# Shizheng-Wen/GAOT-3D

Hardware: AMD Instinct MI355X
Metric: mesh-points/sec fwd+bwd, 500K-pt DrivAerNet++ sample (higher is better)
Workload: dtype bf16; 1 GPU; configs[1]: one 500000-point car-like surface sample, latent 64x64x32, knn k=8 encoder + flipped decoder, C=32 P=2 d=256 h=8 F=1024 L=10 rope, attention dropout 0.1 (training mode), MSE + AdamW step; CSR build and geoembed stats inside the step (a decoder list that is the encoder's with its rows swapped shares the encoder's two lists); points=500000, edges=4000000, edges_decoder=4000000, layers=10, precision=bf16, points_per_gpu=500000, point_order=random

## Files before the change

gaot_3d_amd/csrc/gno.hip:

```cpp
#include <type_traits>

#include "gno_common.h"

namespace {

using namespace gno;

template <int NH, int H>
struct FwdLds {
    static constexpr int KB = H / 32;
    static constexpr int w0 = 0;
    static constexpr int b0 = w0 + IN0P * H;
    static constexpr int wl = b0 + H;
    static constexpr int wL = wl + (NH - 1) * (H * H + H);
    static constexpr int bL = wL + H * 32;
    static constexpr int weights_end = bL + 32;
};

template <int NH, int H, int T, int MODE, class... Nl>
__global__ __launch_bounds__(256, 2) void k_gno_fwd(MlpPtrs mlp, const float* __restrict__ y_pos,
                                                    const float* __restrict__ x_pos, const float* __restrict__ f_y,
                                                    const int* __restrict__ src_s, const int* __restrict__ dst_s,
                                                    const int* __restrict__ rowptr, int64_t E, float* __restrict__ out,
                                                    float* __restrict__ part, Nl... nl_) {
// ... 131 lines not shown
                    acc = __builtin_amdgcn_mfma_f32_32x32x2f32(h[t][kb][r], b, acc, 0, 0, 0);
                }
#pragma unroll
            for (int r = 0; r < 16; ++r) {
                const int el = mfma32_row(r, hf);
                if constexpr (MODE == MODE_KERNELONLY) {
                    stage[(t * 32 + el) * C + l31] = acc[r];
                } else {
                    const int s = ids[(t * 2 + 0) * 32 + el];
                    const float fv = f_y[(int64_t)s * C + l31];
                    stage[(t * 32 + el) * C + l31] = acc[r] * fv;
                }
            }
        }
        wave_lds_fence();
        if (hf < T) {
            segment_walk<C>(stage + hf * 32 * C, C, ids + (hf * 2 + 1) * 32, l31, base + 32 * hf, rowptr, out, part,
                            true);
        }
        wave_lds_fence();
    }
}

__global__ void k_scale_by_inv_deg(const float* __restrict__ gout, const int* __restrict__ rowptr, int64_t Q,
                                   float* __restrict__ gs) {
    const int64_t i = (int64_t)blockIdx.x * blockDim.x + threadIdx.x;
    if (i >= Q * 8) return;
    const int64_t q = i >> 3;
    const int deg = rowptr[q + 1] - rowptr[q];
    const float inv = deg > 0 ? 1.0f / (float)deg : 0.f;
    float4 v = reinterpret_cast<const float4*>(gout)[i];
    reinterpret_cast<float4*>(gs)[i] = make_float4(v.x * inv, v.y * inv, v.z * inv, v.w * inv);
}

__global__ void k_transpose_w(const float* __restrict__ w, int out_dim, int in_dim, float* __restrict__ wt) {
    const int i = blockIdx.x * blockDim.x + threadIdx.x;
    if (i >= out_dim * in_dim) return;
    const int j = i / in_dim, k = i % in_dim;
    wt[k * out_dim + j] = w[i];
}

template <int NH, int H>
struct ParamLayout {
    static constexpr int C = 32;
    static constexpr int w_off(int l) { return l == 0 ? 0 : (H * IN0 + H) + (l - 1) * (H * H + H); }
    static constexpr int b_off(int l) { return w_off(l) + (l == 0 ? H * IN0 : (l == NH ? C * H : H * H)); }
    static constexpr int total = (H * IN0 + H) + (NH - 1) * (H * H + H) + (C * H + C);
};

template <int B, int E, class F>
__device__ __forceinline__ void static_for(F&& f) {
    if constexpr (B < E) {
        f(std::integral_constant<int, B>{});
        static_for<B + 1, E>(f);
    }
}

struct WRsrc {
    __amdgpu_buffer_rsrc_t w[GAOT_MAX_MLP_LAYERS];
    __amdgpu_buffer_rsrc_t wt[GAOT_MAX_MLP_LAYERS];
};
__device__ __forceinline__ float bload(__amdgpu_buffer_rsrc_t r, int voff, int soff) {
// ... 360 lines not shown
        for (int r = 0; r < 16; ++r) wp[PL::w_off(NH) + mfma32_row(r, hf) * H + 32 * wave + l31] = dWL[r];
#pragma unroll
        for (int r = 0; r < 16; ++r)
            if (l31 < IN0) wp[PL::w_off(0) + (32 * wave + mfma32_row(r, hf)) * IN0 + l31] = dW0[r];
        const float t0 = db0 + __shfl_xor(db0, 32, 64);
        if (hf == 0) wp[PL::b_off(0) + 32 * wave + l31] = t0;
        if (wave == 0) {
            const float tl = dbL + __shfl_xor(dbL, 32, 64);
            if (hf == 0) wp[PL::b_off(NH) + l31] = tl;
        }
    }
#pragma unroll
    for (int l = 1; l < NH; ++l) {
#pragma unroll
        for (int r = 0; r < 16; ++r)
            wp[PL::w_off(l) + (32 * wjb + mfma32_row(r, hf)) * H + 32 * wkb + l31] = dWh[l - 1][r];
        if (wkb == 0) {
            const float t = dbh[l - 1] + __shfl_xor(dbh[l - 1], 32, 64);
            if (hf == 0) wp[PL::b_off(l) + 32 * wjb + l31] = t;
        }
    }
}

__global__ __launch_bounds__(256) void k_reduce_params(const float* __restrict__ wpart, int n_waves, int total,
                                                       float* __restrict__ flat) {
    __shared__ float red[4][64];
    const int o = threadIdx.x & 63, sl = threadIdx.x >> 6;
    const int p = blockIdx.x * 64 + o;
    float s = 0.f;
    if (p < total)
        for (int w = sl; w < n_waves; w += 4) s += wpart[(int64_t)w * total + p];
    red[sl][o] = s;
    __syncthreads();
    if (sl == 0 && p < total) flat[p] = ((red[0][o] + red[1][o]) + red[2][o]) + red[3][o];
}

struct ScatterDesc {
    float* dst[2 * GAOT_MAX_MLP_LAYERS];
    int off[2 * GAOT_MAX_MLP_LAYERS + 1];
    int n;
};
__global__ void k_scatter_params(const float* __restrict__ flat, ScatterDesc d) {
    const int p = blockIdx.x * blockDim.x + threadIdx.x;
    if (p >= d.off[d.n]) return;
    int t = 0;
    while (p >= d.off[t + 1]) ++t;
    d.dst[t][p - d.off[t]] = flat[p];
}

int param_total(int nh, int h) { return (h * IN0 + h) + (nh - 1) * (h * h + h) + (32 * h + 32); }

size_t fwd_lds_bytes(int nh, int h, int t) {
    const int weights = IN0P * h + h + (nh - 1) * (h * h + h) + h * 32 + 32;
    return sizeof(float) * (size_t)(weights + 4 * t * 32 * 32) + sizeof(int) * (size_t)(4 * t * 2 * 32);
}
size_t bwd_lds_bytes(int nh, int h, bool coords = false) {
    const int per_wave = nh * 32 * (h + 1) + 32 * (h + 1) + 32 * IN0P + 64;
    return sizeof(float) * (size_t)(4 * per_wave + nh * h + 32 + (coords ? IN0 * h : 0));
}

template <int NH, int H, int MODE>
int launch_fwd(const MlpPtrs& p, const float* y_pos, const float* x_pos, const float* f_y, const float* ttab, const int* src_s,
               const int* dst_s, const int* rowptr, int64_t E, float* out, float* part, hipStream_t st) {
    constexpr int T = 2;
    const size_t lds = fwd_lds_bytes(NH, H, T);
    auto kern = [] {
        if constexpr (MODE == MODE_LINEAR) return k_gno_fwd<NH, H, T, MODE>;
        else return k_gno_fwd<NH, H, T, MODE, NlFwd>;
    }();
    hipError_t e = hipFuncSetAttribute((const void*)kern, hipFuncAttributeMaxDynamicSharedMemorySize, (int)lds);
// ... 45 lines not shown
                               rowptr_src, E, grad_f, part, wpart, nl);
    }
    return GAOT_OK;
}

int bwd_grid(int64_t E) {
    const int64_t n_tiles = ceil_div(E, 32);
    return (int)std::max<int64_t>(1, std::min<int64_t>(ceil_div(n_tiles, 4), 256));
}

bool mlp_supported(const gaot_mlp_t* m, bool backward, int precision = 0) {
    return m && m->channels == 32 && (m->hidden == 64) && m->n_hidden >= 1 &&
           m->n_hidden <= (backward ? (precision == 1 ? 4 : 3) : 4);
}

}

int gaot_gno_fwd_bf16_dispatch(int n_hidden, int mode, const float* const* w, const float* const* b, const float* y_pos,
                               const float* x_pos, const float* f_y, const float* ttab, const int32_t* src_sorted,
                               const int32_t* dst_sorted, const int32_t* rowptr_dst, int64_t num_edges, float* out, float* part,
                               hipStream_t st);

size_t gaot_gno_bwd_bf16_image_bytes(int n_hidden);
int gaot_gno_bwd_bf16_dispatch(int n_hidden, int mode, const float* const* w, const float* const* b, const float* w0t,
                               void* images, const float* y_pos, const float* x_pos, const float* f_y, const float* gs,
                               const int32_t* src_sorted, const int32_t* dst_sorted, const int32_t* rowptr_src,
                               int64_t num_edges, float* grad_f, float* part, float* wpart, float* gcoord, const float* ttab,
                               float* dt, float* part_dt, int grid, hipStream_t st);

extern "C" size_t gaot_gno_fwd_workspace_bytes(int64_t num_edges, int channels) {
    return sizeof(float) * (size_t)(ceil_div(num_edges, 32) * 2 * channels) + 64;
}

namespace {
#define GNO_CHECK(cond, msg)                              \
    do {                                                  \
        if (!(cond)) {                                    \
            gaot_set_error("%s: %s", fn, msg);            \
            return GAOT_ERR_ARG;                          \
        }                                                 \
    } while (0)
int gno_fwd_impl(const char* fn, const gaot_mlp_t* mlp, const float* y_pos, const float* x_pos, const float* f_y,
                 const float* ttab, int mode, const int32_t* src_sorted, const int32_t* dst_sorted, const int32_t* rowptr_dst,
                 int64_t num_edges, int64_t num_queries, float* out, int precision, void* workspace, size_t workspace_bytes,
                 gaot_stream_t stream) {
    GNO_CHECK(mlp, "null mlp");
    if (!mlp_supported(mlp, false)) {
        gaot_set_error("%s: unsupported MLP shape (n_hidden=%d hidden=%d channels=%d)", fn, mlp->n_hidden,
// ... 14 lines not shown
    float* part = (float*)workspace;
    int rc = GAOT_OK;
    if (num_edges > 0) {
        GNO_CHECK(y_pos && x_pos && (f_y || mode == MODE_KERNELONLY) && src_sorted && dst_sorted, "null pointer");
        GNO_CHECK(mode == MODE_LINEAR || ttab, "null t");
        GNO_CHECK(precision == 0 || precision == 1, "precision must be 0 (fp32) or 1 (bf16 matrix cores)");
        if (precision == 1) {
            rc = gaot_gno_fwd_bf16_dispatch(mlp->n_hidden, mode, p.w, p.b, y_pos, x_pos, f_y, ttab, src_sorted, dst_sorted,
                                            rowptr_dst, num_edges, out, part, st);
        } else {
#define GNO_FWD_CASE(NH_, MODE_)                                                                                          \
    case NH_ * 3 + MODE_:                                                                                                 \
        rc = launch_fwd<NH_, 64, MODE_>(p, y_pos, x_pos, f_y, ttab, src_sorted, dst_sorted, rowptr_dst, num_edges, out, part, st); \
        break;
#define GNO_FWD_CASES(NH_) GNO_FWD_CASE(NH_, MODE_LINEAR) GNO_FWD_CASE(NH_, MODE_NONLINEAR) GNO_FWD_CASE(NH_, MODE_KERNELONLY)
            switch (mlp->n_hidden * 3 + mode) {
                GNO_FWD_CASES(1) GNO_FWD_CASES(2) GNO_FWD_CASES(3) GNO_FWD_CASES(4)
            }
#undef GNO_FWD_CASES
#undef GNO_FWD_CASE
        }
        if (rc != GAOT_OK) return rc;
    }
    const int64_t n = num_queries * 8;
    GAOT_KLAUNCH((k_segment_fixup<32>), dim3(segment_fixup_grid(n)), dim3(256), 0, st, rowptr_dst,
                       num_queries, part, out, 1);
    GAOT_LAUNCH_CHECK();
    return GAOT_OK;
}
}

extern "C" int gaot_gno_fwd(const gaot_mlp_t* mlp, const float* y_pos, const float* x_pos, const float* f_y,
                            const int32_t* src_sorted, const int32_t* dst_sorted, const int32_t* rowptr_dst,
                            int64_t num_edges, int64_t num_queries, float* out, int precision, void* workspace,
                            size_t workspace_bytes, gaot_stream_t stream) {
    GAOT_ENTER();
    return gno_fwd_impl("gaot_gno_fwd", mlp, y_pos, x_pos, f_y, nullptr, MODE_LINEAR, src_sorted, dst_sorted, rowptr_dst,
                        num_edges, num_queries, out, precision, workspace, workspace_bytes, stream);
}

extern "C" int gaot_gno_fwd_nl(const gaot_mlp_t* mlp, int mode, const float* y_pos, const float* x_pos, const float* f_y,
                               const float* src_table, const int32_t* src_sorted, const int32_t* dst_sorted,
                               const int32_t* rowptr_dst, int64_t num_edges, int64_t num_queries, float* out, int precision,
                               void* workspace, size_t workspace_bytes, gaot_stream_t stream) {
    GAOT_ENTER();
    GAOT_CHECK_ARG(mode == MODE_NONLINEAR || mode == MODE_KERNELONLY, "mode must be 1 (nonlinear) or 2 (nonlinear_kernelonly)");
    return gno_fwd_impl("gaot_gno_fwd_nl", mlp, y_pos, x_pos, f_y, src_table, mode, src_sorted, dst_sorted, rowptr_dst,
                        num_edges, num_queries, out, precision, workspace, workspace_bytes, stream);
// ... 25 lines not shown
    GNO_CHECK(mlp && grads, "null mlp");
    if (!mlp_supported(mlp, true, precision)) {
        gaot_set_error("%s: unsupported MLP shape (n_hidden=%d hidden=%d channels=%d; four hidden layers in bf16 mode only)", fn,
                       mlp->n_hidden, mlp->hidden, mlp->channels);
        return GAOT_ERR_UNSUPPORTED;
    }
    GNO_CHECK(num_edges >= 0 && num_sources >= 0 && num_queries >= 0, "negative size");
    GNO_CHECK(precision != 1 || (num_sources <= (1 << 24) && num_queries <= (1 << 24)),
                   "bf16 GNO backward: more than 2^24 source or query rows (run the mesh point-sharded or in fp32 mode)");
    GNO_CHECK(precision != 1 || num_edges < ((int64_t)1 << 27),
                   "bf16 GNO backward: 2^27 or more edges in one launch (run the mesh point-sharded or in fp32 mode)");
    const bool nlm = mode != MODE_LINEAR;
    GNO_CHECK(workspace_bytes >= (nlm ? gaot_gno_bwd_nl_workspace_bytes(mlp, num_edges, num_queries)
                                      : gaot_gno_bwd_workspace_bytes(mlp, num_edges, num_queries)), "workspace too small");
    GNO_CHECK(rowptr_src && rowptr_dst, "null rowptr");
    GNO_CHECK(!nlm || num_sources == 0 || dt, "null grad_src_table");
    hipStream_t st = (hipStream_t)stream;
    const int nh = mlp->n_hidden, h = mlp->hidden;
    const int total = param_total(nh, h);
    const int grid = bwd_grid(num_edges);
    const int n_waves = grid;
    float* part = (float*)workspace;
    float* wt = part + ceil_div(num_edges, 16) * 2 * 32;
    float* flat = wt + total;
    float* wpart = flat + total;
    float* gs = wpart + (size_t)grid * total;
    void* images = (void*)(((uintptr_t)(gs + (size_t)num_queries * 32) + 255) & ~(uintptr_t)255);
    float* part_dt = (float*)(((uintptr_t)images + gaot_gno_bwd_bf16_image_bytes(nh) + 255) & ~(uintptr_t)255);
    GNO_CHECK(precision == 0 || precision == 1, "precision must be 0 (fp32) or 1 (bf16 matrix cores)");

    MlpPtrs p, pt;
    int off = 0;
    for (int l = 0; l <= nh; ++l) {
        p.w[l] = mlp->weight[l];
        p.b[l] = mlp->bias[l];
        GNO_CHECK(p.w[l] && p.b[l] && grads->weight[l] && grads->bias[l], "null MLP parameter / gradient");
        const int out_dim = (l == nh) ? 32 : h;
        const int in_dim = (l == 0) ? IN0 : h;
        pt.w[l] = wt + off;
        pt.b[l] = p.b[l];
        if (num_edges > 0)
            GAOT_KLAUNCH(k_transpose_w, dim3((unsigned)ceil_div(out_dim * in_dim, 256)), dim3(256), 0, st, p.w[l],
                               out_dim, in_dim, wt + off);
        off += out_dim * in_dim;
    }
    ScatterDesc sd;
    sd.n = 2 * (nh + 1);
    {
        int o = 0;
        for (int l = 0; l <= nh; ++l) {
            const int out_dim = (l == nh) ? 32 : h;
            const int in_dim = (l == 0) ? IN0 : h;
            sd.dst[2 * l] = grads->weight[l];
            sd.off[2 * l] = o;
            o += out_dim * in_dim;
            sd.dst[2 * l + 1] = grads->bias[l];
            sd.off[2 * l + 1] = o;
            o += out_dim;
        }
        sd.off[sd.n] = o;
    }
    const bool want_gf = mode != MODE_KERNELONLY;
    if (num_edges == 0) {
        hipMemsetAsync(flat, 0, sizeof(float) * total, st);
    } else {
        GNO_CHECK(y_pos && x_pos && grad_out && src_sorted && dst_sorted && (!want_gf || (f_y && grad_f_y)), "null pointer");
        GNO_CHECK(!nlm || ttab, "null src_table");
        const bool cg = gcoord != nullptr;
        GAOT_KLAUNCH(k_scale_by_inv_deg, dim3((unsigned)ceil_div(num_queries * 8, 256)), dim3(256), 0, st, grad_out,
                           rowptr_dst, num_queries, gs);
        int rc = GAOT_OK;
        const NlBwd nl{ttab, dt, part_dt};
        if (precision == 1) {
            rc = gaot_gno_bwd_bf16_dispatch(nh, mode, p.w, p.b, pt.w[0], images, y_pos, x_pos, f_y, gs, src_sorted, dst_sorted,
                                            rowptr_src, num_edges, grad_f_y, part, wpart, gcoord, ttab, dt, part_dt, grid, st);
        } else {
#define GNO_BWD_CASE(NH_, CG_, MODE_)                                                                                       \
    case (NH_ * 2 + CG_) * 3 + MODE_:                                                                                       \
        rc = launch_bwd<NH_, 64, CG_ != 0, MODE_>(p, pt, y_pos, x_pos, f_y, gs, src_sorted, dst_sorted, rowptr_src, num_edges, \
                                                  grad_f_y, part, wpart, gcoord, nl, grid, st);                            \
        break;
#define GNO_BWD_CASES(NH_, CG_) GNO_BWD_CASE(NH_, CG_, MODE_LINEAR) GNO_BWD_CASE(NH_, CG_, MODE_NONLINEAR) GNO_BWD_CASE(NH_, CG_, MODE_KERNELONLY)
            switch ((nh * 2 + (cg ? 1 : 0)) * 3 + mode) {
                GNO_BWD_CASES(1, 0) GNO_BWD_CASES(1, 1) GNO_BWD_CASES(2, 0) GNO_BWD_CASES(2, 1) GNO_BWD_CASES(3, 0) GNO_BWD_CASES(3, 1)
            }
#undef GNO_BWD_CASES
#undef GNO_BWD_CASE
        }
        if (rc != GAOT_OK) return rc;
        GAOT_KLAUNCH(k_reduce_params, dim3((unsigned)ceil_div(total, 64)), dim3(256), 0, st, wpart, n_waves,
                           total, flat);
    }
    GAOT_KLAUNCH(k_scatter_params, dim3((unsigned)ceil_div(total, 256)), dim3(256), 0, st, flat, sd);
    if (num_sources > 0) {
        const int64_t n = num_sources * 8;
        if (want_gf) {
            if (precision == 1)
                GAOT_KLAUNCH((k_segment_fixup<32, 4>), dim3(segment_fixup_grid(n)), dim3(256), 0, st, rowptr_src,
                                   num_sources, part, grad_f_y, 0);
            else
                GAOT_KLAUNCH((k_segment_fixup<32, 5>), dim3(segment_fixup_grid(n)), dim3(256), 0, st, rowptr_src,
                                   num_sources, part, grad_f_y, 0);
        }
        if (nlm) {
            if (precision == 1)
                GAOT_KLAUNCH((k_segment_fixup<NLH, 4>), dim3(segment_fixup_grid(2 * n)), dim3(256), 0, st, rowptr_src,
                                   num_sources, part_dt, dt, 0);
            else
                GAOT_KLAUNCH((k_segment_fixup<NLH, 5>), dim3(segment_fixup_grid(2 * n)), dim3(256), 0, st, rowptr_src,
                                   num_sources, part_dt, dt, 0);
        }
    }
    GAOT_LAUNCH_CHECK();
    return GAOT_OK;
}
#undef GNO_CHECK
}

extern "C" int gaot_gno_bwd(const gaot_mlp_t* mlp, const float* y_pos, const float* x_pos, const float* f_y,
                            const float* grad_out, const int32_t* rowptr_dst, const int32_t* src_sorted,
                            const int32_t* dst_sorted, const int32_t* rowptr_src, int64_t num_edges,
                            int64_t num_sources, int64_t num_queries, float* grad_f_y, const gaot_mlp_grad_t* grads,
                            int precision, void* workspace, size_t workspace_bytes, gaot_stream_t stream) {
    GAOT_ENTER();
    return gno_bwd_impl("gaot_gno_bwd", mlp, y_pos, x_pos, f_y, grad_out, rowptr_dst, src_sorted, dst_sorted, rowptr_src,
                        num_edges, num_sources, num_queries, grad_f_y, grads, nullptr, MODE_LINEAR, nullptr, nullptr, precision,
                        workspace, workspace_bytes, stream);
}

extern "C" int gaot_gno_bwd_coords(const gaot_mlp_t* mlp, const float* y_pos, const float* x_pos, const float* f_y,
                                   const float* grad_out, const int32_t* rowptr_dst, const int32_t* src_sorted,
                                   const int32_t* dst_sorted, const int32_t* rowptr_src, int64_t num_edges,
// ... 23 lines not shown
```

gaot_3d_amd/csrc/gno_bf16.hip:

```cpp
#include <type_traits>

#include "gno_common.h"

namespace {

using namespace gno;
typedef unsigned short bf16_t;

__device__ __forceinline__ short f2bf(float f) { return __builtin_bit_cast(short, (__bf16)f); }

__device__ __forceinline__ void to_frags(const f32x16& v, bf16x8& f0, bf16x8& f1) {
#pragma unroll
    for (int j = 0; j < 8; ++j) {
        f0[j] = f2bf(v[j]);
        f1[j] = f2bf(v[8 + j]);
    }
}
__device__ __forceinline__ constexpr int kmap(int s, int j, int hf) { return 16 * s + 8 * (j >> 2) + 4 * hf + (j & 3); }

template <int NH>
struct FwdLdsB {
    static constexpr int H = 64, KB = 2;
    static constexpr int w0 = 0;
    static constexpr int b0 = w0 + IN0P * H;
// ... 235 lines not shown
    return GAOT_OK;
}

}

int gaot_gno_fwd_bf16_dispatch(int n_hidden, int mode, const float* const* w, const float* const* b, const float* y_pos,
                               const float* x_pos, const float* f_y, const float* ttab, const int32_t* src_sorted,
                               const int32_t* dst_sorted, const int32_t* rowptr_dst, int64_t num_edges, float* out, float* part,
                               hipStream_t st) {
    MlpPtrs p;
    for (int l = 0; l <= n_hidden; ++l) { p.w[l] = w[l]; p.b[l] = b[l]; }
#define GNO_FWDB_CASE(NH_, MODE_) \
    case NH_ * 3 + MODE_: return launch_fwd_b<NH_, MODE_>(p, y_pos, x_pos, f_y, ttab, src_sorted, dst_sorted, rowptr_dst, num_edges, out, part, st);
#define GNO_FWDB_CASES(NH_) GNO_FWDB_CASE(NH_, MODE_LINEAR) GNO_FWDB_CASE(NH_, MODE_NONLINEAR) GNO_FWDB_CASE(NH_, MODE_KERNELONLY)
    if (n_hidden >= 1 && n_hidden <= 4 && mode >= 0 && mode <= 2) switch (n_hidden * 3 + mode) {
        GNO_FWDB_CASES(1) GNO_FWDB_CASES(2) GNO_FWDB_CASES(3) GNO_FWDB_CASES(4)
    }
#undef GNO_FWDB_CASES
#undef GNO_FWDB_CASE
    gaot_set_error("gaot_gno_fwd (bf16): unsupported n_hidden %d / mode %d", n_hidden, mode);
    return GAOT_ERR_UNSUPPORTED;
}

int gaot_gno_bwd3_bf16_launch(int n_hidden, int mode, void* images, const float* w0t, const float* const* w, const float* const* b,
                              const float* y_pos, const float* x_pos, const float* f_y, const float* gs,
                              const int32_t* src_sorted, const int32_t* dst_sorted, const int32_t* rowptr_src,
                              int64_t num_edges, float* grad_f, float* part, float* wpart, float* gcoord, const float* ttab,
                              float* dt, float* part_dt, int grid, hipStream_t st);

size_t gaot_gno_bwd_bf16_image_bytes(int n_hidden) { return (size_t)(n_hidden - 1) * 2 * 8192 + 2 * 4096 + 256; }

int gaot_gno_bwd_bf16_dispatch(int n_hidden, int mode, const float* const* w, const float* const* b, const float* w0t,
                               void* images, const float* y_pos, const float* x_pos, const float* f_y, const float* gs,
                               const int32_t* src_sorted, const int32_t* dst_sorted, const int32_t* rowptr_src,
                               int64_t num_edges, float* grad_f, float* part, float* wpart, float* gcoord, const float* ttab,
                               float* dt, float* part_dt, int grid, hipStream_t st) {
    return gaot_gno_bwd3_bf16_launch(n_hidden, mode, images, w0t, w, b, y_pos, x_pos, f_y, gs, src_sorted, dst_sorted, rowptr_src,
                                     num_edges, grad_f, part, wpart, gcoord, ttab, dt, part_dt, grid, st);
}
```

gaot_3d_amd/csrc/gno_bwd3_bf16.hip:

```cpp
#include <stdlib.h>

#include "gno_common.h"
#include "tile32.h"

namespace {

using namespace gno;

typedef __fp16 h16x2 __attribute__((ext_vector_type(2)));
typedef __bf16 bf16v2 __attribute__((ext_vector_type(2)));

__device__ __host__ __forceinline__ constexpr int kperm(int s, int g, int i) { return 32 * s + 16 * (i >> 2) + 4 * g + (i & 3); }

__device__ __forceinline__ unsigned pk_bf16(float a, float b) {
    const f32v2 t = {a, b};
    return __builtin_bit_cast(unsigned, __builtin_convertvector(t, bf16v2));
}
__device__ __forceinline__ bf16x8 frag_of(const f32x4& lo, const f32x4& hi) {
    return __builtin_bit_cast(bf16x8, make_uint4(pk_bf16(lo[0], lo[1]), pk_bf16(lo[2], lo[3]), pk_bf16(hi[0], hi[1]), pk_bf16(hi[2], hi[3])));
}
__device__ __forceinline__ int tile_off8(int row, int chunk, int half) { return tile_off(row, chunk) + 8 * (half ^ ((row >> 1) & 1)); }
__device__ __forceinline__ void store_frag_rows(char* tile, const bf16x8& f, int s, int n, int g) {
    const uint4 w = __builtin_bit_cast(uint4, f);
    char* half = tile + s * 1024;
// ... 51 lines not shown
    static constexpr int fw(int l) { return (l - 1) * per_hidden; }
    static constexpr int bw(int l) { return (NH - 1) * per_hidden + per_last + (l - 1) * per_hidden; }
    static constexpr bool GIMG = NH >= 4;
    static constexpr int W0S = 80;
    static constexpr int w0t = GIMG ? 0 : img_bytes;
    static constexpr int bias = w0t + 8 * W0S * 4;
    static constexpr int tiles = (bias + (NH * H + C) * 4 + 15) & ~15;
    static constexpr int h(int l) { return l * 2048; }
    static constexpr int dz(int l) { return NH * 2048 + l * 2048; }
    static constexpr int dk = 2 * NH * 2048;
    static constexpr int in = dk + 2048;
    static constexpr int per_wave = in + 512;
    static constexpr int total = tiles + WAVES * per_wave;
};

template <int NH>
struct ParamLayout3 {
    static constexpr int H = 64, C = 32;
    static constexpr int w_off(int l) { return l == 0 ? 0 : (H * IN0 + H) + (l - 1) * (H * H + H); }
    static constexpr int b_off(int l) { return w_off(l) + (l == 0 ? H * IN0 : (l == NH ? C * H : H * H)); }
    static constexpr int total = (H * IN0 + H) + (NH - 1) * (H * H + H) + (C * H + C);
};

__global__ void k_prep_bwd3_images(MlpPtrs mlp, int nh, bf16_t* base) {
    constexpr int H = 64;
    const int per_hidden = 8 * 64 * 8, per_last = 4 * 64 * 8;
    const int total = (nh - 1) * 2 * per_hidden + 2 * per_last;
    for (int idx = blockIdx.x * blockDim.x + threadIdx.x; idx < total; idx += gridDim.x * blockDim.x) {
        int o = idx;
        float v;
        if (o < (nh - 1) * per_hidden) {
            const int l = 1 + o / per_hidden; o %= per_hidden;
            const int i = o & 7, ln = (o >> 3) & 63, fr = o >> 9, s = fr & 1, mb = fr >> 1;
            v = mlp.w[l][(16 * mb + (ln & 15)) * H + kperm(s, ln >> 4, i)];
        } else if ((o -= (nh - 1) * per_hidden) < per_last) {
            const int i = o & 7, ln = (o >> 3) & 63, fr = o >> 9, s = fr & 1, nb = fr >> 1;
            v = mlp.w[nh][(16 * nb + (ln & 15)) * H + kperm(s, ln >> 4, i)];
        } else if ((o -= per_last) < (nh - 1) * per_hidden) {
            const int l = 1 + o / per_hidden; o %= per_hidden;
            const int i = o & 7, ln = (o >> 3) & 63, fr = o >> 9, s = fr & 1, mb = fr >> 1;
            v = mlp.w[l][kperm(s, ln >> 4, i) * H + 16 * mb + (ln & 15)];
        } else {
            o -= (nh - 1) * per_hidden;
            const int i = o & 7, ln = (o >> 3) & 63, mb = o >> 9;
            v = mlp.w[nh][(8 * (ln >> 4) + i) * H + 16 * mb + (ln & 15)];
        }
        base[idx] = f2bf(v);
    }
}

template <int NH, bool CG, int MODE, class... CoordOut>
// ... 438 lines not shown
        }
        attr_set = true;
    }
    if constexpr (MODE == MODE_LINEAR) {
        if constexpr (CG)
            GAOT_KLAUNCH(kern, dim3(grid), dim3(512), lds, st, (const uint4*)images, w0t, p, y_pos, x_pos, f_y, gs, src_s, dst_s,
                         rowptr_src, E, grad_f, part, wpart, gcoord);
        else
            GAOT_KLAUNCH(kern, dim3(grid), dim3(512), lds, st, (const uint4*)images, w0t, p, y_pos, x_pos, f_y, gs, src_s, dst_s,
                         rowptr_src, E, grad_f, part, wpart);
    } else {
        if constexpr (CG)
            GAOT_KLAUNCH(kern, dim3(grid), dim3(512), lds, st, (const uint4*)images, w0t, p, y_pos, x_pos, f_y, gs, src_s, dst_s,
                         rowptr_src, E, grad_f, part, wpart, gcoord, nl);
        else
            GAOT_KLAUNCH(kern, dim3(grid), dim3(512), lds, st, (const uint4*)images, w0t, p, y_pos, x_pos, f_y, gs, src_s, dst_s,
                         rowptr_src, E, grad_f, part, wpart, nl);
    }
    return GAOT_OK;
}

}

int gaot_gno_bwd3_bf16_launch(int n_hidden, int mode, void* images, const float* w0t, const float* const* w, const float* const* b,
                              const float* y_pos, const float* x_pos, const float* f_y, const float* gs,
                              const int32_t* src_sorted, const int32_t* dst_sorted, const int32_t* rowptr_src,
                              int64_t num_edges, float* grad_f, float* part, float* wpart, float* gcoord, const float* ttab,
                              float* dt, float* part_dt, int grid, hipStream_t st) {
    if (n_hidden < 1 || n_hidden > 4 || mode < 0 || mode > 2) {
        gaot_set_error("gaot_gno_bwd (bf16): unsupported n_hidden %d / mode %d", n_hidden, mode);
        return GAOT_ERR_UNSUPPORTED;
    }
    MlpPtrs p;
    for (int l = 0; l <= n_hidden; ++l) { p.w[l] = w[l]; p.b[l] = b[l]; }
    GAOT_KLAUNCH(k_prep_bwd3_images, dim3(32), dim3(256), 0, st, p, n_hidden, (bf16_t*)images);
    const NlBwd nl{ttab, dt, part_dt};
#define GNO_BWD3_CASE(NH_, CG_, MODE_)                                                                                      \
    case (NH_ * 2 + CG_) * 3 + MODE_:                                                                                       \
        return launch_bwd3<NH_, CG_ != 0, MODE_>(images, w0t, p, y_pos, x_pos, f_y, gs, src_sorted, dst_sorted, rowptr_src,   \
                                                 num_edges, grad_f, part, wpart, gcoord, nl, grid, st);
#define GNO_BWD3_CASES(NH_, CG_) GNO_BWD3_CASE(NH_, CG_, MODE_LINEAR) GNO_BWD3_CASE(NH_, CG_, MODE_NONLINEAR) GNO_BWD3_CASE(NH_, CG_, MODE_KERNELONLY)
    switch ((n_hidden * 2 + (gcoord ? 1 : 0)) * 3 + mode) {
        GNO_BWD3_CASES(1, 0) GNO_BWD3_CASES(1, 1) GNO_BWD3_CASES(2, 0) GNO_BWD3_CASES(2, 1)
        GNO_BWD3_CASES(3, 0) GNO_BWD3_CASES(3, 1) GNO_BWD3_CASES(4, 0) GNO_BWD3_CASES(4, 1)
    }
#undef GNO_BWD3_CASES
#undef GNO_BWD3_CASE
    return GAOT_ERR_UNSUPPORTED;
}
```

gaot_3d_amd/csrc/gno_common.h:

```cpp
#pragma once
#include "common.h"

namespace gno {

constexpr int IN0 = 6;
constexpr int IN0P = 8;

template <class T, class... R>
__device__ __forceinline__ T first_arg(T t, R...) { return t; }
template <class T>
__device__ __forceinline__ T last_arg(T t) { return t; }
template <class T, class U, class... R>
__device__ __forceinline__ auto last_arg(T, U u, R... r) { return last_arg(u, r...); }

enum { MODE_LINEAR = 0, MODE_NONLINEAR = 1, MODE_KERNELONLY = 2 };
constexpr int NLH = 64;
struct NlFwd {
    const float* t;
};
struct NlBwd {
    const float* t;
    float* dt;
    float* part_dt;
};

__device__ __forceinline__ void wave_lds_fence() {
    __builtin_amdgcn_fence(__ATOMIC_ACQ_REL, "wavefront");
    __builtin_amdgcn_wave_barrier();
}

struct MlpPtrs {
    const float* w[GAOT_MAX_MLP_LAYERS];
    const float* b[GAOT_MAX_MLP_LAYERS];
};
struct MlpGradPtrs {
    float* w[GAOT_MAX_MLP_LAYERS];
    float* b[GAOT_MAX_MLP_LAYERS];
};

template <int C>
__device__ __forceinline__ void segment_walk(const float* stage, int ld, const int* ids, int c, int64_t tbase,
                                             const int* __restrict__ rowptr, float* __restrict__ out,
                                             float* __restrict__ part, bool mean) {
    const int64_t tile = tbase >> 5;
    int cur = ids[0];
    float sum = 0.f;
    auto flush = [&](int q, float s) {
        if (q < 0) return;
        const int rb = rowptr[q], re = rowptr[q + 1];
        const bool ol = rb < tbase, orr = re > tbase + 32;
        if (!ol && !orr) {
            out[(int64_t)q * C + c] = mean ? s / (float)(re - rb) : s;
        } else if (ol) {
            part[(tile * 2 + 0) * C + c] = s;
        } else {
            part[(tile * 2 + 1) * C + c] = s;
        }
    };
#pragma unroll 4
    for (int e = 0; e < 32; ++e) {
        const int d = ids[e];
        if (d != cur) {
            flush(cur, sum);
            cur = d;
            sum = 0.f;
        }
        if (d >= 0) sum += stage[e * ld + c];
    }
    flush(cur, sum);
}

template <int C, int SHIFT = 5>
__global__ void k_segment_fixup(const int* __restrict__ rowptr, int64_t Q, const float* __restrict__ part,
                                float* __restrict__ out, int mean) {
    static_assert(C % 4 == 0, "four channels per thread");
    constexpr int TPR = C / 4;
    const int64_t n = Q * TPR, stride = (int64_t)gridDim.x * blockDim.x;
    for (int64_t i = (int64_t)blockIdx.x * blockDim.x + threadIdx.x; i < n; i += stride) {
        const int64_t q = i / TPR;
        const int c = (int)(i % TPR) * 4;
        const int rb = rowptr[q], re = rowptr[q + 1];
        float4* o = reinterpret_cast<float4*>(out + q * C + c);
        if (re == rb) {
            *o = make_float4(0.f, 0.f, 0.f, 0.f);
            continue;
        }
        const int t0 = rb >> SHIFT, t1 = (re - 1) >> SHIFT;
        if (t0 == t1) continue;
        float4 s = *reinterpret_cast<const float4*>(part + ((int64_t)t0 * 2 + 1) * C + c);
        for (int t = t0 + 1; t <= t1; ++t) {
            const float4 v = *reinterpret_cast<const float4*>(part + ((int64_t)t * 2 + 0) * C + c);
            s.x += v.x; s.y += v.y; s.z += v.z; s.w += v.w;
        }
        if (mean) {
            const float d = (float)(re - rb);
            s.x /= d; s.y /= d; s.z /= d; s.w /= d;
        }
        *o = s;
    }
}
inline unsigned segment_fixup_grid(int64_t items) {
    const int64_t b = (items + 255) / 256;
    return (unsigned)(b < 1 ? 1 : (b > 4096 ? 4096 : b));
}

}
```

gaot_3d_amd/csrc/rowops.hip:

```cpp
#include "common.h"

namespace {

__global__ void k_rmsnorm_fwd(const float* __restrict__ x, const float* __restrict__ w, float* __restrict__ y,
                              float* __restrict__ rstd, unsigned short* __restrict__ yb, int64_t rows, int d, float eps) {
    const int64_t row = (int64_t)blockIdx.x * 4 + (threadIdx.x >> 6);
    const int lane = threadIdx.x & 63;
    if (row >= rows) return;
    const float4* xr = reinterpret_cast<const float4*>(x + row * d);
    float ss = 0.f;
    for (int i = lane; i < d / 4; i += 64) {
        const float4 v = xr[i];
        ss += v.x * v.x + v.y * v.y + v.z * v.z + v.w * v.w;
    }
    ss = wave_sum(ss);
    const float r = rsqrtf(ss / (float)d + eps);
    if (lane == 0 && rstd) rstd[row] = r;
    float4* yr = reinterpret_cast<float4*>(y + row * d);
    const float4* wr = reinterpret_cast<const float4*>(w);
    for (int i = lane; i < d / 4; i += 64) {
        const float4 v = xr[i], g = wr[i];
        const float4 o = make_float4(v.x * r * g.x, v.y * r * g.y, v.z * r * g.z, v.w * r * g.w);
        yr[i] = o;
        if (yb) {
// ... 162 lines not shown
    const int64_t r1 = (r0 + rows_per_chunk < M) ? r0 + rows_per_chunk : M;
    float4 s = make_float4(0.f, 0.f, 0.f, 0.f);
    if (n < N) {
        int64_t r = r0 + ry;
        for (; r + 24 < r1; r += 32) {
            float4 v[4];
#pragma unroll
            for (int u = 0; u < 4; ++u) v[u] = *reinterpret_cast<const float4*>(x + (r + 8 * u) * ld + n);
#pragma unroll
            for (int u = 0; u < 4; ++u) { s.x += v[u].x; s.y += v[u].y; s.z += v[u].z; s.w += v[u].w; }
        }
        for (; r < r1; r += 8) {
            const float4 v = *reinterpret_cast<const float4*>(x + r * ld + n);
            s.x += v.x; s.y += v.y; s.z += v.z; s.w += v.w;
        }
    }
    sm[ry][cx] = s;
    __syncthreads();
    if (ry == 0 && n < N) {
        float4 t = make_float4(0.f, 0.f, 0.f, 0.f);
#pragma unroll
        for (int j = 0; j < 8; ++j) { t.x += sm[j][cx].x; t.y += sm[j][cx].y; t.z += sm[j][cx].z; t.w += sm[j][cx].w; }
        *reinterpret_cast<float4*>(part + (int64_t)blockIdx.y * N + n) = t;
    }
}

__global__ void k_rope(float* __restrict__ x, int64_t rows, int64_t ld, int col0, int nheads, int HP, int S,
                       const float* __restrict__ freqs, float sign) {
    const int64_t i = (int64_t)blockIdx.x * blockDim.x + threadIdx.x;
    const int64_t n = rows * nheads * HP;
    if (i >= n) return;
    const int p = (int)(i % HP);
    const int hd = (int)((i / HP) % nheads);
    const int64_t row = i / ((int64_t)HP * nheads);
    const float ang = (float)(row % S) * freqs[p];
    float sn, cs;
    sincosf(ang, &sn, &cs);
    sn *= sign;
    float2* px = reinterpret_cast<float2*>(x + row * ld + col0 + hd * (2 * HP) + 2 * p);
    const float2 v = *px;
    *px = make_float2(v.x * cs - v.y * sn, v.y * cs + v.x * sn);
}

__device__ __forceinline__ float sigmoid_f(float v) { return 1.f / (1.f + __expf(-v)); }

__global__ void k_swiglu_fwd(const float* __restrict__ ag, float* __restrict__ u, int64_t rows, int F) {
// ... 299 lines not shown
extern "C" size_t gaot_colsum_workspace_bytes(int64_t M, int64_t N) {
    const int64_t chunks = std::min<int64_t>(256, std::max<int64_t>(1, ceil_div(M, 64)));
    return sizeof(float) * (size_t)(chunks * N) + 64;
}

extern "C" int gaot_colsum(const float* x, int64_t M, int64_t N, int64_t ld, float* out, void* workspace,
                           size_t workspace_bytes, gaot_stream_t stream) {
    GAOT_ENTER();
    GAOT_CHECK_ARG(M >= 0 && N >= 0, "negative size");
    if (N == 0) return GAOT_OK;
    hipStream_t st = (hipStream_t)stream;
    if (M == 0) {
        GAOT_CHECK_ARG(out, "null pointer");
        hipMemsetAsync(out, 0, sizeof(float) * N, st);
        return GAOT_OK;
    }
    GAOT_CHECK_ARG(x && workspace && workspace_bytes >= gaot_colsum_workspace_bytes(M, N), "workspace too small");
    const int64_t chunks = std::min<int64_t>(256, std::max<int64_t>(1, ceil_div(M, 64)));
    const int64_t rpc = ceil_div(M, chunks);
    float* part = (float*)workspace;
    if (N % 4 == 0 && ld % 4 == 0 && ((uintptr_t)x & 15) == 0)
        GAOT_KLAUNCH(k_colsum_part4, dim3((unsigned)ceil_div(N, 128), (unsigned)chunks), dim3(256), 0, st, x, M, N, ld,
                           rpc, part);
    else
        GAOT_KLAUNCH(k_colsum_part, dim3((unsigned)ceil_div(N, 32), (unsigned)chunks), dim3(256), 0, st, x, M, N, ld,
                           rpc, part);
    if (out) GAOT_KLAUNCH(k_reduce_parts, dim3(blocks_for(N, RP_COLS)), dim3(256), 0, st, part, chunks, N, out);
    GAOT_LAUNCH_CHECK();
    return GAOT_OK;
}
extern "C" int64_t gaot_colsum_parts(int64_t M) { return std::min<int64_t>(256, std::max<int64_t>(1, ceil_div(M, 64))); }

namespace {
constexpr int RM_MAX = 64;
struct ReduceTable {
    const float* part[RM_MAX];
    float* out[RM_MAX];
    long long n[RM_MAX];
    int parts[RM_MAX];
    int lanes[RM_MAX];
    int vec[RM_MAX];
    int wide[RM_MAX];
    int blk0[RM_MAX + 1];
    int count;
};
__global__ __launch_bounds__(256) void k_reduce_multi(const ReduceTable t) {
// ... 479 lines not shown
```

Baseline: 25.92 million points/s.

## Fuse GNO backward prologue/epilogue kernels, restructure segment fixup, add narrow colsum

The inverse-degree gradient scaling is merged into the weight-transpose launch (fp32 path) or the bf16 image-prep launch, and the w0 transpose moves into the bf16 prep kernel. The parameter reduce and scatter become one kernel with an unrolled load loop. Segment fixup now stages rowptr in LDS, builds a per-block worklist of rows that span tiles, and batches partial loads. A column-sum kernel for 1-3 column contiguous inputs stages rows through LDS with vector loads. The aim is fewer launches and fewer wasted threads on small memory-bound steps, at the cost of more complex kernels and extra block-level syncs.

Result: no change. 26.07 million points/s, median of 6 (+0.6%).

```diff
diff --git a/gaot_3d_amd/csrc/gno.hip b/gaot_3d_amd/csrc/gno.hip
--- a/gaot_3d_amd/csrc/gno.hip
+++ b/gaot_3d_amd/csrc/gno.hip
@@ -177,22 +177,25 @@
     }
 }
 
-__global__ void k_scale_by_inv_deg(const float* __restrict__ gout, const int* __restrict__ rowptr, int64_t Q,
-                                   float* __restrict__ gs) {
-    const int64_t i = (int64_t)blockIdx.x * blockDim.x + threadIdx.x;
-    if (i >= Q * 8) return;
-    const int64_t q = i >> 3;
-    const int deg = rowptr[q + 1] - rowptr[q];
-    const float inv = deg > 0 ? 1.0f / (float)deg : 0.f;
-    float4 v = reinterpret_cast<const float4*>(gout)[i];
-    reinterpret_cast<float4*>(gs)[i] = make_float4(v.x * inv, v.y * inv, v.z * inv, v.w * inv);
-}
-
-__global__ void k_transpose_w(const float* __restrict__ w, int out_dim, int in_dim, float* __restrict__ wt) {
-    const int i = blockIdx.x * blockDim.x + threadIdx.x;
-    if (i >= out_dim * in_dim) return;
-    const int j = i / in_dim, k = i % in_dim;
-    wt[k * out_dim + j] = w[i];
+struct TransposeTable {
+    const float* w[GAOT_MAX_MLP_LAYERS];
+    int off[GAOT_MAX_MLP_LAYERS + 1];
+    int out_dim[GAOT_MAX_MLP_LAYERS], in_dim[GAOT_MAX_MLP_LAYERS];
+    int n;
+    int blocks;
+};
+__global__ __launch_bounds__(SCALE_THREADS) void k_bwd_prologue(TransposeTable t, float* __restrict__ wt, ScaleJob sj) {
+    if ((int)blockIdx.x >= t.blocks) {
+        scale_by_inv_deg(sj, (int64_t)blockIdx.x - t.blocks);
+        return;
+    }
+    const int p = blockIdx.x * SCALE_THREADS + threadIdx.x;
+    if (p >= t.off[t.n]) return;
+    int l = 0;
+    while (p >= t.off[l + 1]) ++l;
+    const int i = p - t.off[l];
+    const int j = i / t.in_dim[l], k = i % t.in_dim[l];
+    wt[t.off[l] + k * t.out_dim[l] + j] = t.w[l][i];
 }
 
 template <int NH, int H>
@@ -599,30 +602,36 @@
     }
 }
 
-__global__ __launch_bounds__(256) void k_reduce_params(const float* __restrict__ wpart, int n_waves, int total,
-                                                       float* __restrict__ flat) {
-    __shared__ float red[4][64];
-    const int o = threadIdx.x & 63, sl = threadIdx.x >> 6;
-    const int p = blockIdx.x * 64 + o;
-    float s = 0.f;
-    if (p < total)
-        for (int w = sl; w < n_waves; w += 4) s += wpart[(int64_t)w * total + p];
-    red[sl][o] = s;
-    __syncthreads();
-    if (sl == 0 && p < total) flat[p] = ((red[0][o] + red[1][o]) + red[2][o]) + red[3][o];
-}
-
 struct ScatterDesc {
     float* dst[2 * GAOT_MAX_MLP_LAYERS];
     int off[2 * GAOT_MAX_MLP_LAYERS + 1];
     int n;
 };
-__global__ void k_scatter_params(const float* __restrict__ flat, ScatterDesc d) {
-    const int p = blockIdx.x * blockDim.x + threadIdx.x;
-    if (p >= d.off[d.n]) return;
-    int t = 0;
-    while (p >= d.off[t + 1]) ++t;
-    d.dst[t][p - d.off[t]] = flat[p];
+__global__ __launch_bounds__(256) void k_reduce_scatter_params(const float* __restrict__ wpart, int n_waves, ScatterDesc d) {
+    __shared__ float red[4][64];
+    const int total = d.off[d.n];
+    const int o = threadIdx.x & 63, sl = threadIdx.x >> 6;
+    const int p = blockIdx.x * 64 + o;
+    float s = 0.f;
+    if (p < total) {
+        constexpr int B = 16;
+        int w = sl;
+        for (; w + 4 * (B - 1) < n_waves; w += 4 * B) {
+            float v[B];
+#pragma unroll
+            for (int u = 0; u < B; ++u) v[u] = wpart[(int64_t)(w + 4 * u) * total + p];
+#pragma unroll
+            for (int u = 0; u < B; ++u) s += v[u];
+        }
+        for (; w < n_waves; w += 4) s += wpart[(int64_t)w * total + p];
+    }
+    red[sl][o] = s;
+    __syncthreads();
+    if (sl == 0 && p < total) {
+        int t = 0;
+        while (p >= d.off[t + 1]) ++t;
+        d.dst[t][p - d.off[t]] = ((red[0][o] + red[1][o]) + red[2][o]) + red[3][o];
+    }
 }
 
 int param_total(int nh, int h) { return (h * IN0 + h) + (nh - 1) * (h * h + h) + (32 * h + 32); }
@@ -714,8 +723,8 @@
                                hipStream_t st);
 
 size_t gaot_gno_bwd_bf16_image_bytes(int n_hidden);
-int gaot_gno_bwd_bf16_dispatch(int n_hidden, int mode, const float* const* w, const float* const* b, const float* w0t,
-                               void* images, const float* y_pos, const float* x_pos, const float* f_y, const float* gs,
+int gaot_gno_bwd_bf16_dispatch(int n_hidden, int mode, const float* const* w, const float* const* b, float* w0t,
+                               void* images, const float* y_pos, const float* x_pos, const float* f_y, const ScaleJob& sj,
                                const int32_t* src_sorted, const int32_t* dst_sorted, const int32_t* rowptr_src,
                                int64_t num_edges, float* grad_f, float* part, float* wpart, float* gcoord, const float* ttab,
                                float* dt, float* part_dt, int grid, hipStream_t st);
@@ -776,8 +785,7 @@
         }
         if (rc != GAOT_OK) return rc;
     }
-    const int64_t n = num_queries * 8;
-    GAOT_KLAUNCH((k_segment_fixup<32>), dim3(segment_fixup_grid(n)), dim3(256), 0, st, rowptr_dst,
+    GAOT_KLAUNCH((k_segment_fixup<32>), dim3(segment_fixup_grid(num_queries)), dim3(FIX_THREADS), 0, st, rowptr_dst,
                        num_queries, part, out, 1);
     GAOT_LAUNCH_CHECK();
     return GAOT_OK;
@@ -849,27 +857,31 @@
     const int n_waves = grid;
     float* part = (float*)workspace;
     float* wt = part + ceil_div(num_edges, 16) * 2 * 32;
-    float* flat = wt + total;
-    float* wpart = flat + total;
+    float* wpart = wt + 2 * (size_t)total;
     float* gs = wpart + (size_t)grid * total;
     void* images = (void*)(((uintptr_t)(gs + (size_t)num_queries * 32) + 255) & ~(uintptr_t)255);
     float* part_dt = (float*)(((uintptr_t)images + gaot_gno_bwd_bf16_image_bytes(nh) + 255) & ~(uintptr_t)255);
     GNO_CHECK(precision == 0 || precision == 1, "precision must be 0 (fp32) or 1 (bf16 matrix cores)");
 
     MlpPtrs p, pt;
-    int off = 0;
-    for (int l = 0; l <= nh; ++l) {
-        p.w[l] = mlp->weight[l];
-        p.b[l] = mlp->bias[l];
-        GNO_CHECK(p.w[l] && p.b[l] && grads->weight[l] && grads->bias[l], "null MLP parameter / gradient");
-        const int out_dim = (l == nh) ? 32 : h;
-        const int in_dim = (l == 0) ? IN0 : h;
-        pt.w[l] = wt + off;
-        pt.b[l] = p.b[l];
-        if (num_edges > 0)
-            GAOT_KLAUNCH(k_transpose_w, dim3((unsigned)ceil_div(out_dim * in_dim, 256)), dim3(256), 0, st, p.w[l],
-                               out_dim, in_dim, wt + off);
-        off += out_dim * in_dim;
+    TransposeTable tt;
+    tt.n = nh + 1;
+    {
+        int off = 0;
+        for (int l = 0; l <= nh; ++l) {
+            p.w[l] = mlp->weight[l];
+            p.b[l] = mlp->bias[l];
+            GNO_CHECK(p.w[l] && p.b[l] && grads->weight[l] && grads->bias[l], "null MLP parameter / gradient");
+            tt.w[l] = p.w[l];
+            tt.off[l] = off;
+            tt.out_dim[l] = (l == nh) ? 32 : h;
+            tt.in_dim[l] = (l == 0) ? IN0 : h;
+            pt.w[l] = wt + off;
+            pt.b[l] = p.b[l];
+            off += tt.out_dim[l] * tt.in_dim[l];
+        }
+        tt.off[tt.n] = off;
+        tt.blocks = (int)ceil_div(off, SCALE_THREADS);
     }
     ScatterDesc sd;
     sd.n = 2 * (nh + 1);
@@ -888,18 +900,17 @@
         sd.off[sd.n] = o;
     }
     const bool want_gf = mode != MODE_KERNELONLY;
-    if (num_edges == 0) {
-        hipMemsetAsync(flat, 0, sizeof(float) * total, st);
-    } else {
+    if (num_edges > 0) {
         GNO_CHECK(y_pos && x_pos && grad_out && src_sorted && dst_sorted && (!want_gf || (f_y && grad_f_y)), "null pointer");
         GNO_CHECK(!nlm || ttab, "null src_table");
         const bool cg = gcoord != nullptr;
-        GAOT_KLAUNCH(k_scale_by_inv_deg, dim3((unsigned)ceil_div(num_queries * 8, 256)), dim3(256), 0, st, grad_out,
-                           rowptr_dst, num_queries, gs);
+        const ScaleJob sj{grad_out, rowptr_dst, num_queries, gs};
+        if (precision != 1)
+            GAOT_KLAUNCH(k_bwd_prologue, dim3((unsigned)tt.blocks + scale_blocks(num_queries)), dim3(SCALE_THREADS), 0, st, tt, wt, sj);
         int rc = GAOT_OK;
         const NlBwd nl{ttab, dt, part_dt};
         if (precision == 1) {
-            rc = gaot_gno_bwd_bf16_dispatch(nh, mode, p.w, p.b, pt.w[0], images, y_pos, x_pos, f_y, gs, src_sorted, dst_sorted,
+            rc = gaot_gno_bwd_bf16_dispatch(nh, mode, p.w, p.b, wt, images, y_pos, x_pos, f_y, sj, src_sorted, dst_sorted,
                                             rowptr_src, num_edges, grad_f_y, part, wpart, gcoord, ttab, dt, part_dt, grid, st);
         } else {
 #define GNO_BWD_CASE(NH_, CG_, MODE_)                                                                                       \
@@ -915,26 +926,25 @@
 #undef GNO_BWD_CASE
         }
         if (rc != GAOT_OK) return rc;
-        GAOT_KLAUNCH(k_reduce_params, dim3((unsigned)ceil_div(total, 64)), dim3(256), 0, st, wpart, n_waves,
-                           total, flat);
-    }
-    GAOT_KLAUNCH(k_scatter_params, dim3((unsigned)ceil_div(total, 256)), dim3(256), 0, st, flat, sd);
+    }
+    GAOT_KLAUNCH(k_reduce_scatter_params, dim3((unsigned)ceil_div(total, 64)), dim3(256), 0, st, wpart, num_edges > 0 ? n_waves : 0,
+                 sd);
     if (num_sources > 0) {
-        const int64_t n = num_sources * 8;
+        const unsigned fgrid = segment_fixup_grid(num_sources);
         if (want_gf) {
             if (precision == 1)
-                GAOT_KLAUNCH((k_segment_fixup<32, 4>), dim3(segment_fixup_grid(n)), dim3(256), 0, st, rowptr_src,
+                GAOT_KLAUNCH((k_segment_fixup<32, 4>), dim3(fgrid), dim3(FIX_THREADS), 0, st, rowptr_src,
                                    num_sources, part, grad_f_y, 0);
             else
-                GAOT_KLAUNCH((k_segment_fixup<32, 5>), dim3(segment_fixup_grid(n)), dim3(256), 0, st, rowptr_src,
+                GAOT_KLAUNCH((k_segment_fixup<32, 5>), dim3(fgrid), dim3(FIX_THREADS), 0, st, rowptr_src,
                                    num_sources, part, grad_f_y, 0);
         }
         if (nlm) {
             if (precision == 1)
-                GAOT_KLAUNCH((k_segment_fixup<NLH, 4>), dim3(segment_fixup_grid(2 * n)), dim3(256), 0, st, rowptr_src,
+                GAOT_KLAUNCH((k_segment_fixup<NLH, 4>), dim3(fgrid), dim3(FIX_THREADS), 0, st, rowptr_src,
                                    num_sources, part_dt, dt, 0);
             else
-                GAOT_KLAUNCH((k_segment_fixup<NLH, 5>), dim3(segment_fixup_grid(2 * n)), dim3(256), 0, st, rowptr_src,
+                GAOT_KLAUNCH((k_segment_fixup<NLH, 5>), dim3(fgrid), dim3(FIX_THREADS), 0, st, rowptr_src,
                                    num_sources, part_dt, dt, 0);
         }
     }
diff --git a/gaot_3d_amd/csrc/gno_bf16.hip b/gaot_3d_amd/csrc/gno_bf16.hip
--- a/gaot_3d_amd/csrc/gno_bf16.hip
+++ b/gaot_3d_amd/csrc/gno_bf16.hip
@@ -281,19 +281,19 @@
     return GAOT_ERR_UNSUPPORTED;
 }
 
-int gaot_gno_bwd3_bf16_launch(int n_hidden, int mode, void* images, const float* w0t, const float* const* w, const float* const* b,
-                              const float* y_pos, const float* x_pos, const float* f_y, const float* gs,
+int gaot_gno_bwd3_bf16_launch(int n_hidden, int mode, void* images, float* w0t, const float* const* w, const float* const* b,
+                              const float* y_pos, const float* x_pos, const float* f_y, const ScaleJob& sj,
                               const int32_t* src_sorted, const int32_t* dst_sorted, const int32_t* rowptr_src,
                               int64_t num_edges, float* grad_f, float* part, float* wpart, float* gcoord, const float* ttab,
                               float* dt, float* part_dt, int grid, hipStream_t st);
 
 size_t gaot_gno_bwd_bf16_image_bytes(int n_hidden) { return (size_t)(n_hidden - 1) * 2 * 8192 + 2 * 4096 + 256; }
 
-int gaot_gno_bwd_bf16_dispatch(int n_hidden, int mode, const float* const* w, const float* const* b, const float* w0t,
-                               void* images, const float* y_pos, const float* x_pos, const float* f_y, const float* gs,
+int gaot_gno_bwd_bf16_dispatch(int n_hidden, int mode, const float* const* w, const float* const* b, float* w0t,
+                               void* images, const float* y_pos, const float* x_pos, const float* f_y, const ScaleJob& sj,
                                const int32_t* src_sorted, const int32_t* dst_sorted, const int32_t* rowptr_src,
                                int64_t num_edges, float* grad_f, float* part, float* wpart, float* gcoord, const float* ttab,
                                float* dt, float* part_dt, int grid, hipStream_t st) {
-    return gaot_gno_bwd3_bf16_launch(n_hidden, mode, images, w0t, w, b, y_pos, x_pos, f_y, gs, src_sorted, dst_sorted, rowptr_src,
+    return gaot_gno_bwd3_bf16_launch(n_hidden, mode, images, w0t, w, b, y_pos, x_pos, f_y, sj, src_sorted, dst_sorted, rowptr_src,
                                      num_edges, grad_f, part, wpart, gcoord, ttab, dt, part_dt, grid, st);
 }
diff --git a/gaot_3d_amd/csrc/gno_bwd3_bf16.hip b/gaot_3d_amd/csrc/gno_bwd3_bf16.hip
--- a/gaot_3d_amd/csrc/gno_bwd3_bf16.hip
+++ b/gaot_3d_amd/csrc/gno_bwd3_bf16.hip
@@ -97,11 +97,21 @@
     static constexpr int total = (H * IN0 + H) + (NH - 1) * (H * H + H) + (C * H + C);
 };
 
-__global__ void k_prep_bwd3_images(MlpPtrs mlp, int nh, bf16_t* base) {
+constexpr int PREP_BLOCKS = 32;
+__global__ __launch_bounds__(SCALE_THREADS) void k_prep_bwd3_images(MlpPtrs mlp, int nh, bf16_t* base, float* __restrict__ w0t,
+                                                                    ScaleJob sj) {
+    if (blockIdx.x >= PREP_BLOCKS) {
+        scale_by_inv_deg(sj, (int64_t)blockIdx.x - PREP_BLOCKS);
+        return;
+    }
     constexpr int H = 64;
+    if (blockIdx.x < 2) {
+        const int i = blockIdx.x * SCALE_THREADS + threadIdx.x;
+        if (i < H * IN0) w0t[(i % IN0) * H + i / IN0] = mlp.w[0][i];
+    }
     const int per_hidden = 8 * 64 * 8, per_last = 4 * 64 * 8;
     const int total = (nh - 1) * 2 * per_hidden + 2 * per_last;
-    for (int idx = blockIdx.x * blockDim.x + threadIdx.x; idx < total; idx += gridDim.x * blockDim.x) {
+    for (int idx = blockIdx.x * SCALE_THREADS + threadIdx.x; idx < total; idx += PREP_BLOCKS * SCALE_THREADS) {
         int o = idx;
         float v;
         if (o < (nh - 1) * per_hidden) {
@@ -586,8 +596,8 @@
 
 }
 
-int gaot_gno_bwd3_bf16_launch(int n_hidden, int mode, void* images, const float* w0t, const float* const* w, const float* const* b,
-                              const float* y_pos, const float* x_pos, const float* f_y, const float* gs,
+int gaot_gno_bwd3_bf16_launch(int n_hidden, int mode, void* images, float* w0t, const float* const* w, const float* const* b,
+                              const float* y_pos, const float* x_pos, const float* f_y, const ScaleJob& sj,
                               const int32_t* src_sorted, const int32_t* dst_sorted, const int32_t* rowptr_src,
                               int64_t num_edges, float* grad_f, float* part, float* wpart, float* gcoord, const float* ttab,
                               float* dt, float* part_dt, int grid, hipStream_t st) {
@@ -597,7 +607,9 @@
     }
     MlpPtrs p;
     for (int l = 0; l <= n_hidden; ++l) { p.w[l] = w[l]; p.b[l] = b[l]; }
-    GAOT_KLAUNCH(k_prep_bwd3_images, dim3(32), dim3(256), 0, st, p, n_hidden, (bf16_t*)images);
+    GAOT_KLAUNCH(k_prep_bwd3_images, dim3(PREP_BLOCKS + scale_blocks(sj.Q)), dim3(SCALE_THREADS), 0, st, p, n_hidden, (bf16_t*)images,
+                 w0t, sj);
+    const float* gs = sj.gs;
     const NlBwd nl{ttab, dt, part_dt};
 #define GNO_BWD3_CASE(NH_, CG_, MODE_)                                                                                      \
     case (NH_ * 2 + CG_) * 3 + MODE_:                                                                                       \
diff --git a/gaot_3d_amd/csrc/gno_common.h b/gaot_3d_amd/csrc/gno_common.h
--- a/gaot_3d_amd/csrc/gno_common.h
+++ b/gaot_3d_amd/csrc/gno_common.h
@@ -38,6 +38,24 @@
     float* b[GAOT_MAX_MLP_LAYERS];
 };
 
+struct ScaleJob {
+    const float* gout;
+    const int* rowptr_dst;
+    int64_t Q;
+    float* gs;
+};
+constexpr int SCALE_THREADS = 256;
+inline unsigned scale_blocks(int64_t Q) { return (unsigned)((Q * 8 + SCALE_THREADS - 1) / SCALE_THREADS); }
+__device__ __forceinline__ void scale_by_inv_deg(const ScaleJob& j, int64_t block) {
+    const int64_t i = block * SCALE_THREADS + threadIdx.x;
+    if (i >= j.Q * 8) return;
+    const int64_t q = i >> 3;
+    const int deg = j.rowptr_dst[q + 1] - j.rowptr_dst[q];
+    const float inv = deg > 0 ? 1.0f / (float)deg : 0.f;
+    const float4 v = reinterpret_cast<const float4*>(j.gout)[i];
+    reinterpret_cast<float4*>(j.gs)[i] = make_float4(v.x * inv, v.y * inv, v.z * inv, v.w * inv);
+}
+
 template <int C>
 __device__ __forceinline__ void segment_walk(const float* stage, int ld, const int* ids, int c, int64_t tbase,
                                              const int* __restrict__ rowptr, float* __restrict__ out,
@@ -70,38 +88,60 @@
     flush(cur, sum);
 }
 
+constexpr int FIX_THREADS = 256, FIX_ROWS = 64, FIX_MAX_GRID = 8192;
 template <int C, int SHIFT = 5>
-__global__ void k_segment_fixup(const int* __restrict__ rowptr, int64_t Q, const float* __restrict__ part,
-                                float* __restrict__ out, int mean) {
+__global__ __launch_bounds__(FIX_THREADS) void k_segment_fixup(const int* __restrict__ rowptr, int64_t Q,
+                                                               const float* __restrict__ part, float* __restrict__ out, int mean) {
     static_assert(C % 4 == 0, "four channels per thread");
     constexpr int TPR = C / 4;
-    const int64_t n = Q * TPR, stride = (int64_t)gridDim.x * blockDim.x;
-    for (int64_t i = (int64_t)blockIdx.x * blockDim.x + threadIdx.x; i < n; i += stride) {
-        const int64_t q = i / TPR;
-        const int c = (int)(i % TPR) * 4;
-        const int rb = rowptr[q], re = rowptr[q + 1];
-        float4* o = reinterpret_cast<float4*>(out + q * C + c);
-        if (re == rb) {
-            *o = make_float4(0.f, 0.f, 0.f, 0.f);
-            continue;
+    static_assert(FIX_THREADS % TPR == 0 && FIX_ROWS < FIX_THREADS, "whole rows per pass over the worklist; one rowptr load per lane");
+    __shared__ int rp[FIX_ROWS + 1];
+    __shared__ int work[FIX_ROWS];
+    __shared__ int n_work;
+    const int tid = threadIdx.x;
+    for (int64_t q0 = (int64_t)blockIdx.x * FIX_ROWS; q0 < Q; q0 += (int64_t)gridDim.x * FIX_ROWS) {
+        const int rows = (int)((Q - q0 < FIX_ROWS) ? Q - q0 : FIX_ROWS);
+        if (tid == 0) n_work = 0;
+        if (tid <= rows) rp[tid] = rowptr[q0 + tid];
+        __syncthreads();
+        if (tid < rows) {
+            const int rb = rp[tid], re = rp[tid + 1];
+            if (re == rb || (rb >> SHIFT) != ((re - 1) >> SHIFT)) work[atomicAdd(&n_work, 1)] = tid;
         }
-        const int t0 = rb >> SHIFT, t1 = (re - 1) >> SHIFT;
-        if (t0 == t1) continue;
-        float4 s = *reinterpret_cast<const float4*>(part + ((int64_t)t0 * 2 + 1) * C + c);
-        for (int t = t0 + 1; t <= t1; ++t) {
-            const float4 v = *reinterpret_cast<const float4*>(part + ((int64_t)t * 2 + 0) * C + c);
-            s.x += v.x; s.y += v.y; s.z += v.z; s.w += v.w;
+        __syncthreads();
+        const int nw = n_work;
+        for (int k = tid; k < nw * TPR; k += FIX_THREADS) {
+            const int i = work[k / TPR];
+            const int c = (k % TPR) * 4;
+            const int rb = rp[i], re = rp[i + 1];
+            float4* o = reinterpret_cast<float4*>(out + (q0 + i) * C + c);
+            if (re == rb) {
+                *o = make_float4(0.f, 0.f, 0.f, 0.f);
+                continue;
+            }
+            const int t0 = rb >> SHIFT, t1 = (re - 1) >> SHIFT;
+            float4 s = *reinterpret_cast<const float4*>(part + ((int64_t)t0 * 2 + 1) * C + c);
+            for (int t = t0 + 1; t <= t1; t += 4) {
+                float4 p4[4];
+#pragma unroll
+                for (int u = 0; u < 4; ++u)
+                    if (t + u <= t1) p4[u] = *reinterpret_cast<const float4*>(part + ((int64_t)(t + u) * 2 + 0) * C + c);
+#pragma unroll
+                for (int u = 0; u < 4; ++u)
+                    if (t + u <= t1) { s.x += p4[u].x; s.y += p4[u].y; s.z += p4[u].z; s.w += p4[u].w; }
+            }
+            if (mean) {
+                const float d = (float)(re - rb);
+                s.x /= d; s.y /= d; s.z /= d; s.w /= d;
+            }
+            *o = s;
         }
-        if (mean) {
-            const float d = (float)(re - rb);
-            s.x /= d; s.y /= d; s.z /= d; s.w /= d;
-        }
-        *o = s;
+        __syncthreads();
     }
 }
-inline unsigned segment_fixup_grid(int64_t items) {
-    const int64_t b = (items + 255) / 256;
-    return (unsigned)(b < 1 ? 1 : (b > 4096 ? 4096 : b));
+inline unsigned segment_fixup_grid(int64_t rows) {
+    const int64_t b = (rows + FIX_ROWS - 1) / FIX_ROWS;
+    return (unsigned)(b < 1 ? 1 : (b > FIX_MAX_GRID ? FIX_MAX_GRID : b));
 }
 
 }
diff --git a/gaot_3d_amd/csrc/rowops.hip b/gaot_3d_amd/csrc/rowops.hip
--- a/gaot_3d_amd/csrc/rowops.hip
+++ b/gaot_3d_amd/csrc/rowops.hip
@@ -208,6 +208,45 @@
 #pragma unroll
         for (int j = 0; j < 8; ++j) { t.x += sm[j][cx].x; t.y += sm[j][cx].y; t.z += sm[j][cx].z; t.w += sm[j][cx].w; }
         *reinterpret_cast<float4*>(part + (int64_t)blockIdx.y * N + n) = t;
+    }
+}
+
+constexpr int CS_ROWS = 2048;
+template <int N>
+__global__ __launch_bounds__(256) void k_colsum_part_narrow(const float* __restrict__ x, int64_t M, int64_t rows_per_chunk,
+                                                            float* __restrict__ part) {
+    __shared__ __attribute__((aligned(16))) float buf[CS_ROWS * N + 4];
+    __shared__ float sm[8][N];
+    const int tid = threadIdx.x;
+    const int64_t r0 = (int64_t)blockIdx.x * rows_per_chunk;
+    const int64_t r1 = (r0 + rows_per_chunk < M) ? r0 + rows_per_chunk : M;
+    const int col = tid % N, ry = tid / N;
+    float s = 0.f;
+    for (int64_t p0 = r0; p0 < r1; p0 += CS_ROWS) {
+        const int rows = (int)((r1 - p0 < CS_ROWS) ? r1 - p0 : CS_ROWS);
+        const int n = rows * N;
+        const float* src = x + p0 * N;
+        const int sh = (int)(((uintptr_t)src >> 2) & 3);
+        const int head = (4 - sh) & 3;
+        const int nv = n > head ? (n - head) >> 2 : 0;
+        if (tid < head && tid < n) buf[sh + tid] = src[tid];
+        for (int i = tid; i < nv; i += 256)
+            *reinterpret_cast<float4*>(buf + sh + head + 4 * i) = *reinterpret_cast<const float4*>(src + head + 4 * i);
+        for (int i = head + 4 * nv + tid; i < n; i += 256) buf[sh + i] = src[i];
+        __syncthreads();
+        if (tid < 8 * N) {
+#pragma unroll 8
+            for (int r = ry; r < rows; r += 8) s += buf[sh + r * N + col];
+        }
+        __syncthreads();
+    }
+    if (tid < 8 * N) sm[ry][col] = s;
+    __syncthreads();
+    if (tid < N) {
+        float t = 0.f;
+#pragma unroll
+        for (int j = 0; j < 8; ++j) t += sm[j][tid];
+        part[(int64_t)blockIdx.x * N + tid] = t;
     }
 }
 
@@ -553,6 +592,12 @@
     if (N % 4 == 0 && ld % 4 == 0 && ((uintptr_t)x & 15) == 0)
         GAOT_KLAUNCH(k_colsum_part4, dim3((unsigned)ceil_div(N, 128), (unsigned)chunks), dim3(256), 0, st, x, M, N, ld,
                            rpc, part);
+    else if (N == 1 && ld == N)
+        GAOT_KLAUNCH(k_colsum_part_narrow<1>, dim3((unsigned)chunks), dim3(256), 0, st, x, M, rpc, part);
+    else if (N == 2 && ld == N)
+        GAOT_KLAUNCH(k_colsum_part_narrow<2>, dim3((unsigned)chunks), dim3(256), 0, st, x, M, rpc, part);
+    else if (N == 3 && ld == N)
+        GAOT_KLAUNCH(k_colsum_part_narrow<3>, dim3((unsigned)chunks), dim3(256), 0, st, x, M, rpc, part);
     else
         GAOT_KLAUNCH(k_colsum_part, dim3((unsigned)ceil_div(N, 32), (unsigned)chunks), dim3(256), 0, st, x, M, N, ld,
                            rpc, part);
```
